# tkwa/iit

Measured on AMD Instinct MI355X. Metric: IIT (base,source) intervened pairs/sec, IOI GPT-2-small, IOI_ModelPair IIT+strict+behavior step, higher is better.
Workload: dtype bf16; 1 GPU; model=gpt2-small 12L/768d/12H (TL GPT-2 cfg, LNPre, gelu_new, V=50257), global_batch=256, seq_len=16, parallelism=dp1, engine=native, graphs=True

## Files before the change

csrc/kernels.hip:

```cpp
#include "common.h"
#include <stdlib.h>

__global__ void embed_pos_fwd_kernel(const long* __restrict__ tok, const float* __restrict__ WE,
                                     const float* __restrict__ Wpos, float* __restrict__ out, int T, int S, int d) {
  const int t = blockIdx.x;
  if (t >= T) return;
  const long v = tok[t];
  const int s = t % S;
  const float4* e = (const float4*)(WE + v * (long)d);
  const float4* p = (const float4*)(Wpos + (long)s * d);
  float4* o = (float4*)(out + (long)t * d);
  for (int i = threadIdx.x; i < d / 4; i += blockDim.x) {
    float4 a = e[i], b = p[i];
    o[i] = make_float4(a.x + b.x, a.y + b.y, a.z + b.z, a.w + b.w);
  }
}

__global__ void embed_pos_fwd_scalar_kernel(const long* __restrict__ tok, const float* __restrict__ WE,
                                            const float* __restrict__ Wpos, float* __restrict__ out, int T, int S,
                                            int d) {
  const int t = blockIdx.x;
  if (t >= T) return;
  const float* e = WE + tok[t] * (long)d;
  const float* p = Wpos + (long)(t % S) * d;
// ... 252 lines not shown
}

IIT_EXPORT int iit_attn_small_bwd(const void* qkv, const void* dz, const float* lse, void* dqkv,
                                  unsigned long long head_mask, int B, int S, int H, int dh, long ld_qkv, long ld_dz,
                                  float scale, int causal, void* stream) {
  if (S > 64 || dh > 128) return (int)hipErrorInvalidValue;
  const size_t lds = (size_t)(4 * S * (dh + 1) + 2 * S * (S + 1)) * sizeof(float);
  if (lds > kAttnSmallLdsMax) return (int)hipErrorInvalidValue;
  hipLaunchKernelGGL(attn_small_bwd_kernel, dim3(B * H), dim3(64), lds, (hipStream_t)stream, (const __bf16*)qkv,
                     (const __bf16*)dz, lse, (__bf16*)dqkv, head_mask, B, S, H, dh, ld_qkv, ld_dz, scale, causal);
  return hipGetLastError();
}

__device__ __forceinline__ void online_add(float& m, float& s, int& mi, float v, int i) {
  if (v > m) {
    s = s * __expf(m - v) + 1.f;
    m = v;
    mi = i;
  } else if (v != -INFINITY) {
    s += __expf(v - m);
  }
}

__device__ __forceinline__ void online_merge(float& m, float& s, int& mi, float om, float os, int oi) {
  if (om > m || (om == m && oi < mi)) {
    s = os + (m == -INFINITY ? 0.f : s * __expf(m - om));
    m = om;
    mi = oi;
  } else {
    s += (om == -INFINITY ? 0.f : os * __expf(om - m));
  }
}

__global__ __launch_bounds__(1024) void ce_fwd_kernel(const float* __restrict__ logits, long ld, const long* __restrict__ labels,
                                                      float* __restrict__ loss, float* __restrict__ lse_out,
                                                      long* __restrict__ amax, int V) {
  __shared__ float sm_m[16], sm_s[16];
  __shared__ int sm_i[16];
  const int row = blockIdx.x, tid = threadIdx.x, lane = tid & 63, w = tid >> 6;
  const float* x = logits + (long)row * ld;
  float m = -INFINITY, s = 0.f;
  int mi = 0x7fffffff;
  int head = 0;
  if ((((uintptr_t)x) & 15) == 0) {
    const int v4 = V / 4;
    for (int i = tid; i < v4; i += 1024) {
      const float4 q = ((const float4*)x)[i];
      online_add(m, s, mi, q.x, 4 * i);
      online_add(m, s, mi, q.y, 4 * i + 1);
      online_add(m, s, mi, q.z, 4 * i + 2);
      online_add(m, s, mi, q.w, 4 * i + 3);
    }
    head = v4 * 4;
  }
  for (int i = head + tid; i < V; i += 1024) online_add(m, s, mi, x[i], i);
#pragma unroll
  for (int o = 32; o > 0; o >>= 1) {
    const float om = __shfl_xor(m, o, 64), os = __shfl_xor(s, o, 64);
    const int oi = __shfl_xor(mi, o, 64);
    online_merge(m, s, mi, om, os, oi);
  }
  if (lane == 0) { sm_m[w] = m; sm_s[w] = s; sm_i[w] = mi; }
  __syncthreads();
  if (tid == 0) {
    for (int j = 1; j < 16; ++j) online_merge(m, s, mi, sm_m[j], sm_s[j], sm_i[j]);
    const float l = m + __logf(s);
    if (lse_out) lse_out[row] = l;
    if (loss && labels) loss[row] = l - x[labels[row]];
    if (amax) amax[row] = mi;
  }
}

IIT_EXPORT int iit_ce_fwd(const float* logits, long ld, const long* labels, float* loss, float* lse, long* amax, int R,
                          int V, void* stream) {
  hipLaunchKernelGGL(ce_fwd_kernel, dim3(R), dim3(1024), 0, (hipStream_t)stream, logits, ld, labels, loss, lse, amax, V);
  return hipGetLastError();
}

template <typename OUT>
__global__ __launch_bounds__(256) void ce_bwd_kernel(const float* __restrict__ logits, long ld, const long* __restrict__ labels,
                                                     const float* __restrict__ lse, const float* __restrict__ gscale,
                                                     float inv_rows, OUT* __restrict__ out, long ld_out, int V,
                                                     __bf16* __restrict__ out16) {
  const int row = blockIdx.y;
  const int i = blockIdx.x * 256 + threadIdx.x;
  if (i >= ld_out) return;
  float v = 0.f;
  if (i < V) {
    const float p = __expf(logits[(long)row * ld + i] - lse[row]);
    v = (p - (i == labels[row] ? 1.f : 0.f)) * gscale[0] * inv_rows;
  }
  out[(long)row * ld_out + i] = (OUT)v;
  if (out16) out16[(long)row * ld_out + i] = f2bf(v);
}

IIT_EXPORT int iit_ce_bwd(const float* logits, long ld, const long* labels, const float* lse, const float* gscale,
                          float inv_rows, void* out, long ld_out, int R, int V, int out_bf16, void* out16,
                          void* stream) {
  dim3 grid((unsigned)((ld_out + 255) / 256), R);
  if (out_bf16)
    hipLaunchKernelGGL(ce_bwd_kernel<__bf16>, grid, dim3(256), 0, (hipStream_t)stream, logits, ld, labels, lse, gscale,
                       inv_rows, (__bf16*)out, ld_out, V, (__bf16*)nullptr);
  else
    hipLaunchKernelGGL(ce_bwd_kernel<float>, grid, dim3(256), 0, (hipStream_t)stream, logits, ld, labels, lse, gscale,
                       inv_rows, (float*)out, ld_out, V, (__bf16*)out16);
  return hipGetLastError();
}

template <bool VEC>
__global__ __launch_bounds__(256) void ce_bwd16_kernel(const float* __restrict__ logits, long ld,
                                                       const long* __restrict__ labels, const float* __restrict__ lse,
                                                       const float* __restrict__ gscale, float inv_rows,
                                                       __bf16* __restrict__ out16, long ld_out, int V) {
  const int row = blockIdx.y;
  const int c0 = (blockIdx.x * 256 + threadIdx.x) * 8;
  if (c0 >= ld_out) return;
  const float* x = logits + (long)row * ld;
  const float l = lse[row], gs = gscale[0];
  const long lab = labels[row];
  float v[8];
  if (VEC && c0 + 8 <= V) {
    const float4 a = *(const float4*)(x + c0), b = *(const float4*)(x + c0 + 4);
    v[0] = a.x; v[1] = a.y; v[2] = a.z; v[3] = a.w; v[4] = b.x; v[5] = b.y; v[6] = b.z; v[7] = b.w;
  } else {
#pragma unroll
    for (int e = 0; e < 8; ++e) v[e] = c0 + e < V ? x[c0 + e] : 0.f;
  }
  bf16x8 o;
#pragma unroll
  for (int e = 0; e < 8; ++e) {
    const int i = c0 + e;
    float g = 0.f;
    if (i < V) {
      const float p = __expf(v[e] - l);
      g = (p - (i == lab ? 1.f : 0.f)) * gs * inv_rows;
    }
    o[e] = f2bf(g);
  }
  *(bf16x8*)(out16 + (long)row * ld_out + c0) = o;
}

IIT_EXPORT int iit_ce_bwd16(const float* logits, long ld, const long* labels, const float* lse, const float* gscale,
                            float inv_rows, void* out16, long ld_out, int R, int V, void* stream) {
  if (R <= 0 || V <= 0 || ld < V || ld_out < V || ld_out % 8 || ((uintptr_t)out16 & 15)) return (int)hipErrorInvalidValue;
  dim3 grid((unsigned)((ld_out / 8 + 255) / 256), R);
  const bool vec = (((uintptr_t)logits | (uintptr_t)(ld * 4)) & 15) == 0;
  if (vec)
    hipLaunchKernelGGL(ce_bwd16_kernel<true>, grid, dim3(256), 0, (hipStream_t)stream, logits, ld, labels, lse, gscale,
                       inv_rows, (__bf16*)out16, ld_out, V);
  else
    hipLaunchKernelGGL(ce_bwd16_kernel<false>, grid, dim3(256), 0, (hipStream_t)stream, logits, ld, labels, lse,
                       gscale, inv_rows, (__bf16*)out16, ld_out, V);
  return hipGetLastError();
}

struct Span {
  long start4;
  long local4;
  int len4;
  int pad;
};

__global__ __launch_bounds__(256) void sumsq_span_kernel(const float* __restrict__ g, const Span* __restrict__ spans,
                                                         int nspans, float* __restrict__ part, int do_norm,
                                                         int* __restrict__ step, float* __restrict__ gsq) {
  __shared__ float sm[4];
  if (blockIdx.x == 0 && threadIdx.x == 0 && step) step[0] += 1;
  float s = 0.f;
  if (gsq && blockIdx.x == 0 && threadIdx.x < 64) {
    s = gsq[threadIdx.x];
    gsq[threadIdx.x] = 0.f;
  }
  if (!do_norm) return;
  const float4* g4 = (const float4*)g;
  for (int e = blockIdx.x; e < nspans; e += gridDim.x) {
    const Span sp = spans[e];
    for (int i = threadIdx.x; i < sp.len4; i += 256) {
      const float4 v = g4[sp.local4 + i];
      s += (v.x * v.x + v.y * v.y) + (v.z * v.z + v.w * v.w);
    }
  }
  s = wave_sum(s);
  if ((threadIdx.x & 63) == 0) sm[threadIdx.x >> 6] = s;
  __syncthreads();
  if (threadIdx.x == 0) part[blockIdx.x] = sm[0] + sm[1] + sm[2] + sm[3];
// ... 646 lines not shown
  const int lane = threadIdx.x & 63, w = threadIdx.x >> 6;
  const float mw = wave_max(m);
  e = m == -INFINITY ? 0.f : e * __expf(m - mw);
  e = wave_sum(e);
  s = wave_sum(s);
  dba = wave_sum(dba);
  dbl = wave_sum(dbl);
  if (lane == 0) {
    red[0][w] = s; red[1][w] = mw; red[2][w] = e; red[3][w] = dba; red[4][w] = dbl;
  }
  __syncthreads();
  if (threadIdx.x == 0) {
    float M = red[1][0];
    for (int i = 1; i < 4; ++i) M = fmaxf(M, red[1][i]);
    float E = 0.f, S = 0.f, DBA = 0.f, DBL = 0.f;
    for (int i = 0; i < 4; ++i) {
      S += red[0][i];
      E += red[1][i] == -INFINITY ? 0.f : red[2][i] * __expf(red[1][i] - M);
      DBA += red[3][i];
      DBL += red[4][i];
    }
    out[4 * r + 0] = S;
    out[4 * r + 1] = M + __logf(E);
    out[4 * r + 2] = DBA;
    out[4 * r + 3] = DBL;
  }
}

IIT_EXPORT int iit_kl_rows(const float* a, long lda, const float* b, long ldb, int R, int V, float* out, void* stream) {
  if (R <= 0 || V <= 0) return 0;
  hipLaunchKernelGGL(kl_rows_kernel, dim3(R), dim3(256), 0, (hipStream_t)stream, a, lda, b, ldb, V, out);
  return hipGetLastError();
}
```

iit_amd/data/iit_dataset.py:

```python
from __future__ import annotations

from typing import Iterator, Optional, Sequence, Tuple

import numpy as np
import torch
from torch.utils.data import DataLoader, Dataset, Subset

from ..config import DEVICE


def _gather_fn(ds):
    if hasattr(ds, "gather"):
        return ds.gather
    if isinstance(ds, Subset):
        inner = _gather_fn(ds.dataset)
        if inner is None:
            return None
        table = torch.as_tensor(list(ds.indices), dtype=torch.long)
        cache = {}

        def f(idx, _inner=inner, _table=table, _cache=cache):
            dev = idx.device
            t = _cache.get(dev)
            if t is None:
                t = _cache[dev] = _table.to(dev)
            return _inner(t.index_select(0, idx))

        return f
    return None


def _dist_info() -> Tuple[int, int]:
    if torch.distributed.is_available() and torch.distributed.is_initialized():
        return torch.distributed.get_rank(), torch.distributed.get_world_size()
    return 0, 1


def loader_epoch_permutation(n: int) -> torch.Tensor:
    torch.empty((), dtype=torch.int64).random_()
    seed = int(torch.empty((), dtype=torch.int64).random_().item())
    g = torch.Generator()
    g.manual_seed(seed)
    return torch.randperm(n, generator=g)


class IITDataset(Dataset):
    def __init__(self, base_data, ablation_data, seed: int = 0, every_combination: bool = False, device=DEVICE):
        self.base_data = base_data
        self.ablation_data = ablation_data
        self.seed = seed
        self.every_combination = every_combination
        self.device = device
        self._pair_table: Optional[Tuple[np.ndarray, np.ndarray]] = None

    def pair_indices(self, index: int) -> Tuple[int, int]:
        if self.every_combination:
            n_abl = len(self.ablation_data)
            return index // n_abl, index % n_abl
        rng = np.random.default_rng(self.seed * 1000000 + index)
        base = rng.choice(len(self.base_data))
        abl = rng.choice(len(self.ablation_data))
        return int(base), int(abl)
# ... 27 lines not shown

    @staticmethod
    def collate_fn(batch, device=DEVICE):
        base, abl = zip(*batch)
        return (IITDataset.get_encoded_input_from_torch_input(base, device),
                IITDataset.get_encoded_input_from_torch_input(abl, device))

    def supports_device_loader(self) -> bool:
        return _gather_fn(self.base_data) is not None and _gather_fn(self.ablation_data) is not None

    def make_loader(self, batch_size: int, num_workers: int = 0, shuffle: bool = True, fast: Optional[bool] = None):
        if fast is None:
            fast = self.supports_device_loader()
        if fast:
            return DeviceIITLoader(self, batch_size, shuffle=shuffle)
        return DataLoader(self, batch_size=batch_size, shuffle=shuffle, num_workers=num_workers,
                          collate_fn=lambda b: self.collate_fn(b, self.device))


class DeviceIITLoader:

    def __init__(self, dataset: IITDataset, batch_size: int, shuffle: bool = True, drop_last: bool = False,
                 device=None):
        self.dataset = dataset
        self.batch_size = batch_size
        self.shuffle = shuffle
        self.drop_last = drop_last
        self.rank, self.world = _dist_info()
        self.device = torch.device(device) if device is not None else torch.device(dataset.device)
        self._base_gather = _gather_fn(dataset.base_data)
        self._abl_gather = _gather_fn(dataset.ablation_data)
        self._unique = isinstance(dataset, IITUniqueDataset)
        self._tables = None

    def _device_tables(self):
        if self._tables is None:
            if self._unique:
                self._tables = (None, None)
            else:
                b, a = self.dataset.pair_table()
                self._tables = (torch.as_tensor(b).to(self.device), torch.as_tensor(a).to(self.device))
        return self._tables

    @property
    def global_batch(self) -> int:
        return self.batch_size * self.world

    def __len__(self) -> int:
        n = len(self.dataset)
        gb = self.global_batch
        if self.drop_last or (self.world > 1 and 0 < n % gb < self.world):
            return n // gb
        return (n + gb - 1) // gb

    def __iter__(self) -> Iterator:
        n = len(self.dataset)
        perm = loader_epoch_permutation(n) if self.shuffle else torch.arange(n)
        if self.device.type == "cuda":
            perm = perm.pin_memory().to(self.device, non_blocking=True)
        else:
            perm = perm.to(self.device)
        base_t, abl_t = self._device_tables()
        gb = self.global_batch
        for start in range(0, n, gb):
            chunk = perm[start:start + gb]
            if chunk.numel() < gb and self.drop_last:
                break
            if self.world > 1:
                if chunk.numel() < self.world:
                    break
                chunk = torch.tensor_split(chunk, self.world)[self.rank]
            if self._unique:
                yield self._base_gather(chunk)
            else:
                yield (self._base_gather(base_t.index_select(0, chunk)),
                       self._abl_gather(abl_t.index_select(0, chunk)))


class IITUniqueDataset(IITDataset):

    def __getitem__(self, index):
        return self.base_data[index]

    def __len__(self) -> int:
        return len(self.base_data)

    @staticmethod
    def collate_fn(batch, device=DEVICE):
        return IITDataset.get_encoded_input_from_torch_input(batch, device)

    def supports_device_loader(self) -> bool:
        return _gather_fn(self.base_data) is not None

    def make_loader(self, batch_size: int, num_workers: int = 0, shuffle: bool = True, fast: Optional[bool] = None):
        if fast is None:
            fast = self.supports_device_loader()
        if fast:
            return DeviceIITLoader(self, batch_size, shuffle=shuffle)
        return DataLoader(self, batch_size=batch_size, shuffle=shuffle, num_workers=num_workers,
                          collate_fn=lambda b: self.collate_fn(b, self.device))


def train_test_split(dataset, test_size: float = 0.2, random_state: Optional[int] = None):
    n = len(dataset)
    split = int(n * test_size)
    if random_state is None:
# ... 4 lines not shown
```

iit_amd/model_pairs/ioi_model_pair.py:

```python
from __future__ import annotations

import numpy as np
import torch
import torch.nn.functional as F
from torch import Tensor

from ..config import DEVICE
from ..core import index as index_mod
from ..core.metric import MetricStore, MetricStoreCollection, MetricType, PerTokenMetricStore
from .base_model_pair import _ll_nodes_of
from .strict_iit_model_pair import StrictIITModelPair


def _last(t: Tensor, seq_dim_present: bool) -> Tensor:
    return t[:, -1] if seq_dim_present else t


class IOI_ModelPair(StrictIITModelPair):
    def __init__(self, hl_model, ll_model, corr, training_args=None):
        super().__init__(hl_model, ll_model, corr, training_args=training_args)
        defaults = {"next_token": False, "non_ioi_thresh": 0.65, "use_per_token_check": False}
        self.training_args = {**defaults, **self.training_args}
        self.next_token = bool(self.training_args["next_token"])

    def ll_logits_mode(self) -> str:
        return "full" if (self.next_token or not self.native()) else "last"

    def hl_run_kwargs(self):
        if self.native() and not self.next_token and getattr(self.hl_model, "supports_last_only", False):
            return {"last_only": True}
        return {}

    @property
    def loss_fn(self):
        if self._loss_fn_override is not None:
            return self._loss_fn_override
        return self.per_token_weighted_cross_entropy

    @loss_fn.setter
    def loss_fn(self, value):
        self._loss_fn_override = value

    def per_token_weighted_cross_entropy(self, output: Tensor, target: Tensor) -> Tensor:
        output = output.float()
        if output.dim() == 2:
            if target.dim() == 3 or (target.dim() == 2 and not target.dtype.is_floating_point):
                target = target[:, -1]
            if target.dtype.is_floating_point and target.dim() == 2:
                target = target.argmax(-1) if bool((target.sum(-1) == 1).all()) else target
            if not target.dtype.is_floating_point:
                from ..ops import cross_entropy
                return cross_entropy(output, target)
            return F.cross_entropy(output, target)
        if self.next_token:
            B, S, V = output.shape
            if target.dtype.is_floating_point:
                per = -(target * F.log_softmax(output, -1)).sum(-1)
            else:
                per = F.cross_entropy(output.reshape(B * S, V), target.reshape(B * S), reduction="none").view(B, S)
            w = torch.ones(S, device=output.device)
            w[-1] = 10
            return (per * w).sum() / (w.sum() * B)
        return F.cross_entropy(output[:, -1, :], target[:, -1])

    @staticmethod
    def get_label_idxs():
        return index_mod.Ix[:, -1]

    @staticmethod
    def make_test_metrics():
        return MetricStoreCollection([
            MetricStore("val/iit_loss", MetricType.LOSS),
            MetricStore("val/IIA", MetricType.ACCURACY),
            MetricStore("val/accuracy", MetricType.ACCURACY),
            PerTokenMetricStore("val/per_token_accuracy"),
        ])

    @staticmethod
    def _hl_label(hl_output: Tensor) -> Tensor:
        return torch.argmax(hl_output[:, -1] if hl_output.dim() == 3 else hl_output, dim=-1)

    def fast_hl_label(self, base_x: Tensor, ablation_x: Tensor, hl_node):
        from ..tasks.ioi.ioi_hl import IOI_HL
        hl = self.hl_model
        if not (self.native() and self.training_args.get("fast_hl", True) and type(hl) is IOI_HL
                and base_x.is_cuda and base_x.dtype == torch.long and ablation_x.dtype == torch.long):
            return None
        from ..ops import hip_kernels as K
        node = K.IOI_HL_NODES.get(hl_node.name)
        if node is None or not (hl_node.index is None or hl_node.index.is_everything()):
            return None
        if base_x.dim() != 2 or base_x.shape != ablation_x.shape or base_x.shape[1] > 64:
            return None
        if any(hp.is_live for hp in hl.hook_dict.values()):
            return None
        nm = hl.name_mover_head
# ... 65 lines not shown
```

iit_amd/model_pairs/strict_iit_model_pair.py:

```python
from __future__ import annotations

from ..core.metric import MetricStore, MetricStoreCollection, MetricType
from ..core.nodes import LLNode
from ..utils import node_picker
from .iit_behavior_model_pair import IITBehaviorModelPair


class StrictIITModelPair(IITBehaviorModelPair):
    def __init__(self, hl_model, ll_model, corr, training_args=None):
        defaults = {
            "batch_size": 256,
            "lr": 0.001,
            "num_workers": 0,
            "use_single_loss": False,
            "iit_weight": 1.0,
            "behavior_weight": 1.0,
            "strict_weight": 1.0,
            "clip_grad_norm": 1.0,
        }
        super().__init__(hl_model, ll_model, corr=corr, training_args={**defaults, **(training_args or {})})
        self.nodes_not_in_circuit = node_picker.get_nodes_not_in_circuit(self.ll_model, self.corr)

    @staticmethod
    def make_train_metrics():
        return MetricStoreCollection([
            MetricStore("train/iit_loss", MetricType.LOSS),
            MetricStore("train/behavior_loss", MetricType.LOSS),
            MetricStore("train/strict_loss", MetricType.LOSS),
        ])

    def sample_ll_node(self) -> LLNode:
        return self.rng.choice(self.nodes_not_in_circuit)

    def get_strict_loss_over_batch(self, base_input, ablation_input, ll_node: LLNode, loss_fn):
        base_x, base_y = base_input[0], base_input[1]
        out = self.ll_paired_intervention(base_x, ablation_input[0], [ll_node])
        if out is None:
            self.ll_cache = self.ll_source_cache(ablation_input[0], [ll_node])
            out = self.ll_intervened_forward(base_x, [ll_node])
        if out.dim() > 1 and out.shape[0] == 1:
            return loss_fn(out, base_y)
        return loss_fn(out.squeeze() if 1 in out.shape else out, base_y)

    def run_train_step(self, base_input, ablation_input, loss_fn, optimizer):
        args = self.training_args
        hl_node = self.sample_hl_name()

        def iit():
            return self.get_IIT_loss_over_batch(base_input, ablation_input, hl_node, loss_fn) * args["iit_weight"]

        if args["use_single_loss"]:
            ll_node = self.sample_ll_node()

            def total():
                parts = {"iit": iit(),
                         "strict": self.get_strict_loss_over_batch(base_input, ablation_input, ll_node, loss_fn)
                         * args["strict_weight"],
                         "behavior": self.get_behaviour_loss_over_batch(base_input, loss_fn) * args["behavior_weight"]}
                return parts["iit"] + parts["behavior"] + parts["strict"], parts

            _, parts = self.run_phase(("single", hl_node.name, ll_node.name, repr(ll_node.index)), total, optimizer,
                                      self.step_on_loss)
            return {"train/iit_loss": parts["iit"], "train/behavior_loss": parts["behavior"],
                    "train/strict_loss": parts["strict"]}
        iit_loss = self.run_phase(("iit", hl_node.name), iit, optimizer, self.step_on_loss)
        ll_node = self.sample_ll_node()
        strict_loss = self.run_phase(
            ("strict", ll_node.name, repr(ll_node.index)),
            lambda: self.get_strict_loss_over_batch(base_input, ablation_input, ll_node, loss_fn) * args["strict_weight"],
            optimizer, self.step_on_loss)
        behavior_loss = self.run_phase(
            ("behavior",), lambda: self.get_behaviour_loss_over_batch(base_input, loss_fn) * args["behavior_weight"],
            optimizer, self.step_on_loss)
        return {"train/iit_loss": iit_loss, "train/behavior_loss": behavior_loss, "train/strict_loss": strict_loss}
```

iit_amd/ops/__init__.py:

```python
from __future__ import annotations

from typing import Optional

import torch

from .torch_ops import TorchOps, gelu_new

_TORCH_OPS_CACHE = {}


def _torch_ops(dtype):
    ops = _TORCH_OPS_CACHE.get(dtype)
    if ops is None:
        ops = _TORCH_OPS_CACHE[dtype] = TorchOps(dtype)
    return ops


def hip_supported(cfg) -> bool:
    return (cfg.positional_embedding_type == "standard" and cfg.normalization_type in ("LN", "LNPre", None)
            and not cfg.gated_mlp and (cfg.n_key_value_heads in (None, cfg.n_heads))
            and not cfg.parallel_attn_mlp and not cfg.final_rms
            and cfg.act_fn in ("gelu_new", "gelu_fast", "gelu_pytorch_tanh", "gelu", "relu"))


def select_ops(model, backend: Optional[str] = None):
    cfg = model.cfg
    dtype = cfg.dtype
    on_gpu = next(model.parameters()).is_cuda
    if backend is None:
        from .. import config as _config
        env = _config.backend()
        backend = "hip" if (on_gpu and dtype == torch.bfloat16 and env == "hip" and hip_supported(cfg)) else "torch"
    if backend == "torch":
        return _torch_ops(dtype)
    if backend == "hip":
        if not on_gpu:
            raise RuntimeError("hip op backend requires the model on a GPU")
        from .hip_ops import get_hip_ops
        return get_hip_ops(model)
    if backend in ("hip32", "hip32x"):
        if not on_gpu:
            raise RuntimeError(f"{backend} op backend requires the model on a GPU")
        from .hip32_ops import get_hip32_ops, get_hip32x_ops
        return (get_hip32_ops if backend == "hip32" else get_hip32x_ops)(model)
    raise ValueError(f"unknown op backend {backend}")


def cross_entropy(logits: torch.Tensor, target: torch.Tensor) -> torch.Tensor:
    if logits.is_cuda and logits.dim() == 2 and not target.dtype.is_floating_point:
        from .hip_ops import cross_entropy as _hip_ce
        return _hip_ce(logits, target)
    return torch.nn.functional.cross_entropy(logits.float(), target)
```

iit_amd/ops/hip_kernels.py:

```python
from __future__ import annotations

import ctypes
import math
import os
from typing import Optional, Sequence

import numpy as np
import torch

from . import build as _build

c_void_p, c_long, c_int, c_float, c_ull = ctypes.c_void_p, ctypes.c_long, ctypes.c_int, ctypes.c_float, ctypes.c_ulonglong

EPI_BF16, EPI_BF16_BIAS3, EPI_F32_RESID, EPI_GELU, EPI_DGELU, EPI_F32_ACC, EPI_F32_ACC_QKV, EPI_F32_STORE = range(8)
EPI_GELU_ERF = 8
EPI_DGELU_ERF = 9
MODE_NN, MODE_AKM, MODE_BKM, MODE_AF32, MODE_BF32 = 0, 1, 2, 4, 8

_LIB = None
GEMM_GROUP_M = 4
GEMM_DUAL_GROUP_M = 2

_SIGS = {
    "iit_gemm": [c_void_p] * 10 + [c_long] * 5 + [c_int] * 12 + [c_void_p],
    "iit_gemm_f32": [c_void_p] * 6 + [c_long] * 4 + [c_int] * 7 + [c_void_p],
    "iit_gemm_f32_ok": [c_void_p] * 6 + [c_long] * 4 + [c_int] * 7,
    "iit_attn_f32_lds": [c_int] * 3,
    "iit_attn_f32_waves": [c_int] * 3,
    "iit_attn_f32_ok": [c_void_p] * 4 + [c_int] * 4,
    "iit_attn_f32_fwd": [c_void_p] * 6 + [c_int] * 4 + [c_float, c_int, c_void_p],
    "iit_attn_f32_bwd": [c_void_p] * 9 + [c_int] * 4 + [c_float, c_int, c_void_p],
    "iit_gemm_glds": [c_void_p] * 8 + [c_long] * 5 + [c_int] * 8 + [c_void_p] * 4,
    "iit_gemm_glds_ok": [c_void_p] * 5 + [c_long] * 5 + [c_int] * 9,
    "iit_gemm_glds_sm": [c_void_p] * 8 + [c_long] * 5 + [c_int] * 8 + [c_void_p] * 3 + [c_int] + [c_void_p] * 3,
    "iit_embed_pos_fwd": [c_void_p, c_void_p, c_void_p, c_void_p, c_int, c_int, c_int, c_void_p],
    "iit_embed_pos_bwd": [c_void_p, c_void_p, c_void_p, c_void_p, c_int, c_int, c_int, c_void_p],
    "iit_ln_fwd": [c_void_p] * 7 + [c_int, c_int, c_float, c_ull, c_int, c_int, c_void_p],
    "iit_ln_bwd": [c_void_p, c_int, c_void_p, c_int] + [c_void_p] * 10 + [c_int, c_int, c_int, c_ull, c_int, c_void_p],
    "iit_ln_bwd_part_rows": [],
    "iit_attn_small_fwd": [c_void_p] * 4 + [c_ull, c_int, c_int, c_int, c_int, c_long, c_long, c_long, c_float, c_int,
                                            c_void_p],
    "iit_attn_small_bwd": [c_void_p] * 4 + [c_ull, c_int, c_int, c_int, c_int, c_long, c_long, c_float, c_int, c_void_p],
    "iit_attn_mfma_fwd": [c_void_p] * 4 + [c_ull, c_int, c_int, c_int, c_int, c_long, c_long, c_long, c_float, c_int,
                                           c_void_p],
    "iit_attn_mfma_fwd_pair": [c_void_p] * 4 + [c_ull, c_int, c_int, c_int, c_int, c_long, c_long, c_long, c_float,
                                                c_int, c_void_p, c_int, c_ull, c_void_p],
    "iit_attn_mfma_bwd": [c_void_p] * 4 + [c_ull, c_int, c_int, c_int, c_int, c_long, c_long, c_float, c_int, c_void_p],
    "iit_attn_mfma_fwd_spec": [c_void_p] * 3 + [c_int] * 4 + [c_long, c_long, c_float, c_int, c_int, c_void_p,
                                                               c_void_p],
    "iit_attn_mfma_bwd_spec": [c_void_p] * 4 + [c_int] * 4 + [c_long, c_long, c_float, c_int, c_void_p, c_void_p],
    "iit_ce_fwd": [c_void_p, c_long, c_void_p, c_void_p, c_void_p, c_void_p, c_int, c_int, c_void_p],
    "iit_ce_bwd": [c_void_p, c_long, c_void_p, c_void_p, c_void_p, c_float, c_void_p, c_long, c_int, c_int, c_int,
                   c_void_p, c_void_p],
    "iit_gemm_glds_edge_ok": [c_void_p] * 4 + [c_long] * 3 + [c_int] * 6,
    "iit_gemm_glds_edge": [c_void_p] * 4 + [c_long] * 3 + [c_int] * 7 + [c_void_p, c_void_p, c_int, c_void_p],
    "iit_gemm_edge_plan": [c_int, c_int, c_long, c_int, c_int, c_void_p],
    "iit_ce_bwd16": [c_void_p, c_long, c_void_p, c_void_p, c_void_p, c_float, c_void_p, c_long, c_int, c_int, c_void_p],
    "iit_adam_flat": [c_void_p] * 6 + [c_int, c_void_p, c_int] + [c_float] * 6 + [c_void_p] * 3
                     + [c_void_p, c_int, c_void_p, c_void_p],
    "iit_sumsq_2d": [c_void_p, c_long, c_int, c_int, c_void_p, c_void_p],
    "iit_kl_rows": [c_void_p, c_long, c_void_p, c_long, c_int, c_int, c_void_p, c_void_p],
    "iit_adam_span_size": [],
    "iit_sumsq_spans": [c_void_p, c_void_p, c_int, c_void_p, c_int, c_int, c_void_p, c_void_p],
    "iit_adam_spans": [c_void_p] * 6 + [c_int, c_void_p] + [c_float] * 6 + [c_void_p] * 4,
    "iit_gelu_fwd": [c_void_p, c_long, c_void_p, c_long, c_int, c_int, c_int, c_void_p],
    "iit_shadow_refresh": [c_void_p, c_int, c_void_p],
    "iit_shadow_desc_size": [],
    "iit_colsum_accum": [c_void_p, c_int, c_long, c_void_p, c_int, c_int, c_void_p],
    "iit_dgelu": [c_void_p, c_void_p, c_void_p, c_long, c_int, c_void_p],
    "iit_add_bf16": [c_void_p, c_long, c_void_p, c_long, c_void_p, c_long, c_void_p, c_int, c_int, c_void_p],
    "iit_device_sync": [],
    "iit_zero_chunks": [c_void_p, c_void_p, c_int, c_void_p],
    "iit_zero_ranges": [c_void_p, c_void_p, c_void_p, c_int, c_void_p],
    "iit_colsum_multi": [c_void_p] * 6 + [c_int, c_void_p],
    "iit_rms_fwd": [c_void_p, c_int, c_void_p, c_void_p, c_void_p, c_int, c_int, c_float, c_void_p],
    "iit_rms_bwd": [c_void_p, c_void_p, c_int, c_void_p, c_void_p, c_void_p, c_void_p, c_int, c_int, c_void_p],
    "iit_rms_bwd_res": [c_void_p, c_void_p, c_int, c_void_p, c_void_p, c_void_p, c_void_p, c_void_p, c_int, c_int,
                        c_void_p],
    "iit_rotary": [c_void_p, c_long, c_long, c_long, c_void_p, c_void_p, c_void_p] + [c_int] * 8 + [c_void_p],
    "iit_swiglu_fwd": [c_void_p, c_void_p, c_void_p, c_long, c_void_p],
    "iit_swiglu_bwd": [c_void_p] * 5 + [c_long, c_void_p],
    "iit_swiglu_splice_fwd": [c_void_p] * 4 + [c_long, c_void_p, c_void_p],
    "iit_sparse_pair": [c_void_p, c_long, c_long, c_void_p, c_int, c_void_p],
    "iit_gemm_dual_set_group_m": [c_int],
    "iit_swiglu_splice_bwd": [c_void_p] * 5 + [c_long, c_void_p, c_void_p],
    "iit_embed_splice_fwd": [c_void_p, c_void_p, c_long, c_void_p, c_void_p, c_long, c_int, c_void_p, c_void_p],
    "iit_embed_splice_bwd": [c_void_p, c_void_p, c_int, c_void_p, c_long, c_long, c_int, c_void_p, c_void_p],
    "iit_flash_fwd": [c_void_p] * 3 + [c_void_p, c_void_p, c_void_p, c_void_p, c_void_p, c_void_p, c_ull] + [c_int] * 5
                     + [c_float, c_int, c_void_p, c_void_p],
    "iit_flash_bwd": [c_void_p] * 3 + [c_void_p] * 11 + [c_ull] + [c_int] * 5 + [c_float, c_int, c_void_p, c_void_p],
# ... 851 lines not shown
    _check(lib().iit_embed_splice_fwd(_p(tokens), _p(W16), W16.stride(0), _p(out), _p(src), T, d, spec_ptr,
                                      _stream()), "embed_splice_fwd")


def embed_splice_bwd(tokens, dout, grad, spec_ptr):
    T, d = tokens.numel(), dout.shape[-1]
    _check(lib().iit_embed_splice_bwd(_p(tokens), _p(dout), int(dout.dtype == torch.float32), _p(grad),
                                      grad.stride(0), T, d, spec_ptr, _stream()), "embed_splice_bwd")


def swiglu_splice_bwd(dpost, gate, up, dgate, dup, spec_ptr):
    _check(lib().iit_swiglu_splice_bwd(_p(dpost), _p(gate), _p(up), _p(dgate), _p(dup), gate.numel(), spec_ptr,
                                       _stream()), "swiglu_splice_bwd")


def swiglu_bwd(dpost, gate, up, dgate, dup):
    _check(lib().iit_swiglu_bwd(_p(dpost), _p(gate), _p(up), _p(dgate), _p(dup), gate.numel(), _stream()),
           "swiglu_bwd")


def ce_fwd(logits, ld, labels, loss, lse, amax, R, V):
    if CHECK_BOUNDS:
        _bounds("ce_fwd", ("logits", logits, R, V, ld))
    _check(lib().iit_ce_fwd(_p(logits), ld, _p(labels), _p(loss), _p(lse), _p(amax), R, V, _stream()), "ce_fwd")


def ce_bwd(logits, ld, labels, lse, gscale, inv_rows, out, ld_out, R, V, out16=None):
    if CHECK_BOUNDS:
        _bounds("ce_bwd", ("logits", logits, R, V, ld), ("out", out, R, V, ld_out))
    _check(lib().iit_ce_bwd(_p(logits), ld, _p(labels), _p(lse), _p(gscale), inv_rows, _p(out), ld_out, R, V,
                            int(out.dtype == torch.bfloat16), _p(out16), _stream()), "ce_bwd")


def ce_bwd16(logits, ld, labels, lse, gscale, inv_rows, out16, ld_out, R, V):
    assert logits.dtype == torch.float32 and out16.dtype == torch.bfloat16 and gscale.dtype == torch.float32
    if CHECK_BOUNDS:
        _bounds("ce_bwd16", ("logits", logits, R, V, ld), ("out16", out16, R, ld_out, ld_out))
    _check(lib().iit_ce_bwd16(_p(logits), ld, _p(labels), _p(lse), _p(gscale), inv_rows, _p(out16), ld_out, R, V,
                              _stream()), "ce_bwd16")


def colsum_accum(x, ld, out, T, N):
    if CHECK_BOUNDS:
        _bounds("colsum", ("x", x, T, N, ld), ("out", out, 1, N, N))
    _check(lib().iit_colsum_accum(_p(x), int(x.dtype == torch.float32), ld, _p(out), T, N, _stream()), "colsum")


def colsum_vec_ok(x, ld, out, N) -> bool:
    cpt = 4 if x.dtype == torch.float32 else 8
    return (x.dtype in (torch.float32, torch.bfloat16) and out.dtype == torch.float32 and N % cpt == 0
            and ld % cpt == 0 and x.data_ptr() % 16 == 0)


def colsum_multi(items):
    import numpy as np
    if not items:
        return
    xs = np.array([it[0].data_ptr() for it in items], dtype=np.int64)
    outs = np.array([it[2].data_ptr() for it in items], dtype=np.int64)
    lds = np.array([it[1] for it in items], dtype=np.int64)
    Ts = np.array([it[3] for it in items], dtype=np.int32)
    Ns = np.array([it[4] for it in items], dtype=np.int32)
    f32s = np.array([int(it[0].dtype == torch.float32) for it in items], dtype=np.int32)
    if CHECK_BOUNDS:
        for x, ld, out, T, N in items:
            _bounds("colsum_multi", ("x", x, T, N, ld), ("out", out, 1, N, N))
    _check(lib().iit_colsum_multi(xs.ctypes.data, outs.ctypes.data, lds.ctypes.data, Ts.ctypes.data, Ns.ctypes.data,
                                  f32s.ctypes.data, len(items), _stream()), "colsum_multi")


def colsum3_accum(x, ld, outs, T, N):
    for i, o in enumerate(outs):
# ... 70 lines not shown
```

iit_amd/ops/hip_ops.py:

```python
from __future__ import annotations

import math
import os
from typing import Optional, Sequence

import torch
from torch.autograd import Function

from ..engine import grad_hooks
from . import hip_kernels as K
from .gemm_dispatch import gemm, gemm_pair
from .torch_ops import TorchOps, act_fn

BF16 = torch.bfloat16
F32 = torch.float32


def _pad8(n: int) -> int:
    return (n + 7) // 8 * 8


def _grad_slot(p: Optional[torch.Tensor]) -> Optional[torch.Tensor]:
    if p is None or not p.requires_grad:
        return None
# ... 1036 lines not shown
        return _mlp_out_forward(ctx, pre, post, W, b, w, ldw, resid, b_in, erf)

    @staticmethod
    def backward(ctx, gy):
        if gy is None:
            return (None,) * 9
        x2, pre2 = ctx.saved_tensors
        W, b, b_in = ctx.params
        lead, Kd, N = ctx.meta
        T = x2.shape[0]
        g16 = _bf16_of(gy)
        g2 = _aligned_rows(g16, T, N)
        ldg = g2.stride(0)
        dpre = xspec = gbi = None
        if ctx.needs_input_grad[0]:
            dpre = torch.empty(T, Kd, dtype=BF16, device=g2.device)
            gbi = _grad_slot(b_in)
            xspec = dict(A=g2, B=ctx.w, C=dpre, M=T, N=Kd, K=N, lda=ldg, ldb=ctx.ldw, ldc=Kd, mode=K.MODE_NN,
                         epi=K.EPI_DGELU_ERF if ctx.erf else K.EPI_DGELU, aux=pre2, ldc2=pre2.stride(0), colsum=gbi)
        store, (gW,) = _wgrad_slots(True, W)
        gb = _grad_slot(b)
        bs = _wgrad_tail(ctx, xspec, x2, g2, ldg, (W,), *_wgrad_rows(gW, Kd, N), store, gb)
        if dpre is not None:
            dpre = dpre.view(*lead, Kd)
            if gbi is not None:
                dpre._iit_bias_sum = (dpre.data_ptr(), dpre._version, id(b_in))
        _bias_tail(bs, gb, g2, ldg, (b,), (W,))
        return dpre, None, None, None, None, None, gy, None, None


class CrossEntropyFn(Function):

    @staticmethod
    def forward(ctx, logits, labels, handle=None):
        ctx.set_materialize_grads(False)
        R, V = logits.shape
        if logits.stride(1) != 1:
            logits = logits.contiguous()
        ld = logits.stride(0)
        loss = torch.empty(R, dtype=F32, device=logits.device)
        lse = torch.empty(R, dtype=F32, device=logits.device)
        lab = labels.contiguous()
        K.ce_fwd(logits, ld, lab, loss, lse, None, R, V)
        ctx.save_for_backward(logits, lab, lse)
        ctx.only16 = handle is not None
        return loss.mean()

    @staticmethod
    def backward(ctx, g):
        if g is None:
            return None, None, None
        logits, lab, lse = ctx.saved_tensors
        R, V = logits.shape
        ld = logits.stride(0)
        ldo = _pad8(V)
        buf16 = torch.empty(R, ldo, dtype=BF16, device=logits.device)
        gs = g.reshape(1).float().contiguous()
        if ctx.only16:
            K.ce_bwd16(logits, ld, lab, lse, gs, 1.0 / R, buf16, ldo, R, V)
            return None, None, buf16[:, :V]
        buf = torch.empty(R, ldo, dtype=F32, device=logits.device)
        K.ce_bwd(logits, ld, lab, lse, gs, 1.0 / R, buf, ldo, R, V, out16=buf16)
        res = buf[:, :V]
        _set_bf16_twin(res, buf16[:, :V])
        return res, None, None


def _grad16_handle(logits: torch.Tensor) -> Optional[torch.Tensor]:
    tag = getattr(logits, "_iit_grad16", None)
    if tag is None or tag[0] != logits.data_ptr() or tag[1] != logits._version or tag[2].shape != logits.shape:
        return None
    if not (torch.is_grad_enabled() and tag[2].requires_grad) or logits._backward_hooks or logits.retains_grad:
        return None
    if os.environ.get("IIT_CE_BF16_ONLY", "1") == "0":
        return None
    return tag[2]


def cross_entropy(logits: torch.Tensor, labels: torch.Tensor) -> torch.Tensor:
    logits = logits.float()
    handle = _grad16_handle(logits) if logits.dim() == 2 else None
    if handle is not None:
        logits._iit_grad16 = None
        return CrossEntropyFn.apply(logits.detach(), labels, handle)
    return CrossEntropyFn.apply(logits, labels)




class Paired:

    __slots__ = ("base", "full", "f32")

    def __init__(self, base: torch.Tensor, full: torch.Tensor, f32=None):
        self.base, self.full, self.f32 = base, full, f32

    def resid_operands(self):
        if self.f32 is not None:
            return self.f32
        return self.base, self.full.float().contiguous()

    @property
    def nb(self) -> int:
        return self.base.shape[0]

    @property
    def src(self) -> torch.Tensor:
        return self.full[self.nb:]


class EmbedPosPairFn(EmbedPosFn):
    @staticmethod
    def forward(ctx, tokens, W_E, W_pos, tokens_full, box):
        ctx.set_materialize_grads(False)
        B2, S = tokens_full.shape
        d = W_E.shape[1]
        B = tokens.shape[0]
        out = torch.empty(B2, S, d, dtype=F32, device=tokens.device)
# ... 495 lines not shown
```

iit_amd/tasks/ioi/ioi_dataset.py:

```python
from __future__ import annotations

import random
from typing import Dict, List, Optional, Sequence

import torch
from torch.utils.data import Dataset

from ...config import DEVICE
from .ioi_config import NAMES, NOUNS, TEMPLATES, vocabulary_words
from .tokenizer import SyntheticTokenizer


def default_tokenizer() -> SyntheticTokenizer:
    return SyntheticTokenizer(vocabulary_words())


class IOIDataset(Dataset):
    def __init__(self, tokenizer=None, templates: Optional[List[str]] = None, names: Optional[List[str]] = None,
                 nouns: Optional[Dict[str, List[str]]] = None, num_samples: int = 1000, symmetric: bool = False,
                 prepend_bos: bool = True, seed: int = 42, device=None):
        self.tokenizer = tokenizer if tokenizer is not None else default_tokenizer()
        self.prepend_bos = prepend_bos
        self.templates = list(templates) if templates is not None else list(TEMPLATES)
        self.names = list(names) if names is not None else list(NAMES)
# ... 42 lines not shown
    @staticmethod
    def get_default_names():
        return list(NAMES)

    @staticmethod
    def get_default_templates():
        return list(TEMPLATES)

    @staticmethod
    def get_default_nouns():
        return {k: list(v) for k, v in NOUNS.items()}


class IOIDatasetWrapper(IOIDataset):

    def __init__(self, *args, label_format: str = "index", **kwargs):
        if label_format not in ("index", "onehot"):
            raise ValueError("label_format must be 'index' or 'onehot'")
        self.label_format = label_format
        super().__init__(*args, **kwargs)

    def _labels(self, y: torch.Tensor) -> torch.Tensor:
        if self.label_format == "onehot":
            return torch.nn.functional.one_hot(y, num_classes=self.tokenizer.vocab_size).float()
        return y

    def __getitem__(self, idx):
        p = self.prompts[idx]
        return p[:-1], self._labels(p[1:]), self.io_ids[idx:idx + 1]

    def token_ids(self) -> torch.Tensor:
        return torch.unique(self.prompts[:, :-1])

    def gather(self, idx: torch.Tensor):
        p = self.prompts.index_select(0, idx.to(self.prompts.device))
        return p[:, :-1], self._labels(p[:, 1:]), self.io_ids.index_select(0, idx.to(self.prompts.device))[:, None]
```

Measured before the change: 16990 pairs/s.

## Fuse CE mean and loss weighting into kernels; fuse pair batch gather

The cross-entropy forward gains a mean variant. The last block to finish, found through an atomic ticket, reduces the per-row losses and applies the loss weight, which replaces a separate mean launch and weight multiply. The backward folds the weight into the bf16 gradient kernel. A new kernel gathers base and source prompts, labels and IO ids for a batch in one launch, replacing several index_select and slicing ops per batch. The ticket-based last-block reduction adds cross-block atomic ordering to get right and a shared per-device ticket buffer.

```diff
diff --git a/csrc/kernels.hip b/csrc/kernels.hip
--- a/csrc/kernels.hip
+++ b/csrc/kernels.hip
@@ -308,9 +308,11 @@
   }
 }
 
+template <bool MEAN>
 __global__ __launch_bounds__(1024) void ce_fwd_kernel(const float* __restrict__ logits, long ld, const long* __restrict__ labels,
                                                       float* __restrict__ loss, float* __restrict__ lse_out,
-                                                      long* __restrict__ amax, int V) {
+                                                      long* __restrict__ amax, int V, float weight,
+                                                      float* __restrict__ mean_out, int* __restrict__ ticket) {
   __shared__ float sm_m[16], sm_s[16];
   __shared__ int sm_i[16];
   const int row = blockIdx.x, tid = threadIdx.x, lane = tid & 63, w = tid >> 6;
@@ -342,14 +344,59 @@
     for (int j = 1; j < 16; ++j) online_merge(m, s, mi, sm_m[j], sm_s[j], sm_i[j]);
     const float l = m + __logf(s);
     if (lse_out) lse_out[row] = l;
-    if (loss && labels) loss[row] = l - x[labels[row]];
+    if constexpr (MEAN) {
+      __hip_atomic_store(loss + row, l - x[labels[row]], __ATOMIC_RELAXED, __HIP_MEMORY_SCOPE_AGENT);
+    } else {
+      if (loss && labels) loss[row] = l - x[labels[row]];
+    }
     if (amax) amax[row] = mi;
+  }
+  if constexpr (MEAN) {
+    __shared__ int is_last;
+    const int R = gridDim.x;
+    if (tid == 0) {
+      asm volatile("s_waitcnt vmcnt(0)" ::: "memory");
+      const int last = __hip_atomic_fetch_add(ticket, 1, __ATOMIC_RELAXED, __HIP_MEMORY_SCOPE_AGENT) == R - 1;
+      if (last) __hip_atomic_store(ticket, 0, __ATOMIC_RELAXED, __HIP_MEMORY_SCOPE_AGENT);
+      is_last = last;
+    }
+    __syncthreads();
+    if (!is_last) return;
+    float acc = 0.f;
+    for (int base = 0; base < R; base += 4096) {
+      float v[4];
+#pragma unroll
+      for (int e = 0; e < 4; ++e) {
+        const int i = base + e * 1024 + tid;
+        v[e] = i < R ? __hip_atomic_load(loss + i, __ATOMIC_RELAXED, __HIP_MEMORY_SCOPE_AGENT) : 0.f;
+      }
+      acc += (v[0] + v[1]) + (v[2] + v[3]);
+    }
+#pragma unroll
+    for (int o = 32; o > 0; o >>= 1) acc += __shfl_xor(acc, o, 64);
+    if (lane == 0) sm_s[w] = acc;
+    __syncthreads();
+    if (w == 0) {
+      float t = lane < 16 ? sm_s[lane] : 0.f;
+#pragma unroll
+      for (int o = 8; o > 0; o >>= 1) t += __shfl_xor(t, o, 64);
+      if (lane == 0) mean_out[0] = t / (float)R * weight;
+    }
   }
 }
 
 IIT_EXPORT int iit_ce_fwd(const float* logits, long ld, const long* labels, float* loss, float* lse, long* amax, int R,
                           int V, void* stream) {
-  hipLaunchKernelGGL(ce_fwd_kernel, dim3(R), dim3(1024), 0, (hipStream_t)stream, logits, ld, labels, loss, lse, amax, V);
+  hipLaunchKernelGGL(ce_fwd_kernel<false>, dim3(R), dim3(1024), 0, (hipStream_t)stream, logits, ld, labels, loss, lse,
+                     amax, V, 1.f, (float*)nullptr, (int*)nullptr);
+  return hipGetLastError();
+}
+
+IIT_EXPORT int iit_ce_fwd_mean(const float* logits, long ld, const long* labels, float* loss, float* lse, int R, int V,
+                               float weight, float* mean_out, int* ticket, void* stream) {
+  if (R <= 0 || V <= 0 || ld < V || !labels || !loss || !mean_out || !ticket) return (int)hipErrorInvalidValue;
+  hipLaunchKernelGGL(ce_fwd_kernel<true>, dim3(R), dim3(1024), 0, (hipStream_t)stream, logits, ld, labels, loss, lse,
+                     (long*)nullptr, V, weight, mean_out, ticket);
   return hipGetLastError();
 }
 
@@ -386,13 +433,14 @@
 template <bool VEC>
 __global__ __launch_bounds__(256) void ce_bwd16_kernel(const float* __restrict__ logits, long ld,
                                                        const long* __restrict__ labels, const float* __restrict__ lse,
-                                                       const float* __restrict__ gscale, float inv_rows,
-                                                       __bf16* __restrict__ out16, long ld_out, int V) {
+                                                       const float* __restrict__ gscale, float weight,
+                                                       float inv_rows, __bf16* __restrict__ out16, long ld_out,
+                                                       int V) {
   const int row = blockIdx.y;
   const int c0 = (blockIdx.x * 256 + threadIdx.x) * 8;
   if (c0 >= ld_out) return;
   const float* x = logits + (long)row * ld;
-  const float l = lse[row], gs = gscale[0];
+  const float l = lse[row], gs = gscale[0] * weight;
   const long lab = labels[row];
   float v[8];
   if (VEC && c0 + 8 <= V) {
@@ -417,16 +465,16 @@
 }
 
 IIT_EXPORT int iit_ce_bwd16(const float* logits, long ld, const long* labels, const float* lse, const float* gscale,
-                            float inv_rows, void* out16, long ld_out, int R, int V, void* stream) {
+                            float inv_rows, void* out16, long ld_out, int R, int V, float weight, void* stream) {
   if (R <= 0 || V <= 0 || ld < V || ld_out < V || ld_out % 8 || ((uintptr_t)out16 & 15)) return (int)hipErrorInvalidValue;
   dim3 grid((unsigned)((ld_out / 8 + 255) / 256), R);
   const bool vec = (((uintptr_t)logits | (uintptr_t)(ld * 4)) & 15) == 0;
   if (vec)
     hipLaunchKernelGGL(ce_bwd16_kernel<true>, grid, dim3(256), 0, (hipStream_t)stream, logits, ld, labels, lse, gscale,
-                       inv_rows, (__bf16*)out16, ld_out, V);
+                       weight, inv_rows, (__bf16*)out16, ld_out, V);
   else
     hipLaunchKernelGGL(ce_bwd16_kernel<false>, grid, dim3(256), 0, (hipStream_t)stream, logits, ld, labels, lse,
-                       gscale, inv_rows, (__bf16*)out16, ld_out, V);
+                       gscale, weight, inv_rows, (__bf16*)out16, ld_out, V);
   return hipGetLastError();
 }
 
@@ -1139,3 +1187,41 @@
   hipLaunchKernelGGL(kl_rows_kernel, dim3(R), dim3(256), 0, (hipStream_t)stream, a, lda, b, ldb, V, out);
   return hipGetLastError();
 }
+
+struct PairGatherSide {
+  const long* tab;
+  const long* prompts;
+  const long* io;
+  long* x;
+  long* y;
+  long* iv;
+  long N;
+};
+
+__global__ __launch_bounds__(256) void pair_batch_gather_kernel(const long* __restrict__ perm, int n, long ntab, int S1,
+                                                                const PairGatherSide a, const PairGatherSide b) {
+  const PairGatherSide& sd = blockIdx.y == 0 ? a : b;
+  const int e = blockIdx.x * 256 + threadIdx.x;
+  if (e >= n * S1) return;
+  const int r = e / S1, c = e - r * S1, S = S1 - 1;
+  const long p = perm[r];
+  if ((unsigned long)p >= (unsigned long)ntab) return;
+  const long i = sd.tab[p];
+  if ((unsigned long)i >= (unsigned long)sd.N) return;
+  const long v = sd.prompts[i * S1 + c];
+  if (c < S) sd.x[(long)r * S + c] = v;
+  if (c > 0) sd.y[(long)r * S + c - 1] = v;
+  if (c == 0) sd.iv[r] = sd.io[i];
+}
+
+IIT_EXPORT int iit_pair_batch_gather(const long* perm, int n, long ntab, int S1, const long* tab_b, const long* prompts_b,
+                                     const long* io_b, long Nb, const long* tab_a, const long* prompts_a,
+                                     const long* io_a, long Na, long* xb, long* yb, long* ivb, long* xa, long* ya,
+                                     long* iva, void* stream) {
+  if (n <= 0) return 0;
+  if (S1 < 2 || (long)n * S1 > 0x7fffffffL) return (int)hipErrorInvalidValue;
+  const PairGatherSide a{tab_b, prompts_b, io_b, xb, yb, ivb, Nb}, b{tab_a, prompts_a, io_a, xa, ya, iva, Na};
+  hipLaunchKernelGGL(pair_batch_gather_kernel, dim3((unsigned)(((long)n * S1 + 255) / 256), 2), dim3(256), 0,
+                     (hipStream_t)stream, perm, n, ntab, S1, a, b);
+  return hipGetLastError();
+}
diff --git a/iit_amd/data/iit_dataset.py b/iit_amd/data/iit_dataset.py
--- a/iit_amd/data/iit_dataset.py
+++ b/iit_amd/data/iit_dataset.py
@@ -28,6 +28,21 @@
 
         return f
     return None
+
+
+def _pair_gather_side(ds, table: torch.Tensor):
+    while isinstance(ds, Subset):
+        table = torch.as_tensor(list(ds.indices), dtype=torch.long).to(table.device).index_select(0, table)
+        ds = ds.dataset
+    ops = ds.pair_gather_operands() if hasattr(ds, "pair_gather_operands") else None
+    if ops is None:
+        return None
+    prompts, io_ids = ops
+    if prompts.device != table.device or prompts.dtype != torch.long or io_ids.dtype != torch.long:
+        return None
+    if table.numel() and not (0 <= int(table.min()) and int(table.max()) < prompts.shape[0]):
+        raise IndexError("pair table points outside the dataset")
+    return table.contiguous(), prompts.contiguous(), io_ids.contiguous()
 
 
 def _dist_info() -> Tuple[int, int]:
@@ -121,6 +136,7 @@
         self._abl_gather = _gather_fn(dataset.ablation_data)
         self._unique = isinstance(dataset, IITUniqueDataset)
         self._tables = None
+        self._sides = None
 
     def _device_tables(self):
         if self._tables is None:
@@ -131,6 +147,18 @@
                 self._tables = (torch.as_tensor(b).to(self.device), torch.as_tensor(a).to(self.device))
         return self._tables
 
+    def _pair_sides(self):
+        if self._sides is None:
+            sides = None
+            if self.device.type == "cuda" and not self._unique:
+                ds = self.dataset
+                sides = tuple(_pair_gather_side(d, t) for d, t in zip((ds.base_data, ds.ablation_data),
+                                                                      self._device_tables()))
+                if None in sides or sides[0][1].shape[1] != sides[1][1].shape[1]:
+                    sides = None
+            self._sides = (sides,)
+        return self._sides[0]
+
     @property
     def global_batch(self) -> int:
         return self.batch_size * self.world
@@ -150,6 +178,7 @@
         else:
             perm = perm.to(self.device)
         base_t, abl_t = self._device_tables()
+        sides = self._pair_sides()
         gb = self.global_batch
         for start in range(0, n, gb):
             chunk = perm[start:start + gb]
@@ -161,6 +190,9 @@
                 chunk = torch.tensor_split(chunk, self.world)[self.rank]
             if self._unique:
                 yield self._base_gather(chunk)
+            elif sides is not None:
+                from ..ops import hip_kernels
+                yield hip_kernels.pair_batch_gather(chunk, sides[0], sides[1], sides[0][1].shape[1])
             else:
                 yield (self._base_gather(base_t.index_select(0, chunk)),
                        self._abl_gather(abl_t.index_select(0, chunk)))
diff --git a/iit_amd/model_pairs/ioi_model_pair.py b/iit_amd/model_pairs/ioi_model_pair.py
--- a/iit_amd/model_pairs/ioi_model_pair.py
+++ b/iit_amd/model_pairs/ioi_model_pair.py
@@ -41,7 +41,13 @@
     def loss_fn(self, value):
         self._loss_fn_override = value
 
-    def per_token_weighted_cross_entropy(self, output: Tensor, target: Tensor) -> Tensor:
+    def per_token_weighted_cross_entropy(self, output: Tensor, target: Tensor, weight=None) -> Tensor:
+        if weight is not None:
+            if output.dim() == 2 and output.is_cuda and (
+                    not target.dtype.is_floating_point and target.dim() in (1, 2)):
+                from ..ops import cross_entropy
+                return cross_entropy(output.float(), target[:, -1] if target.dim() == 2 else target, weight=weight)
+            return self.per_token_weighted_cross_entropy(output, target) * weight
         output = output.float()
         if output.dim() == 2:
             if target.dim() == 3 or (target.dim() == 2 and not target.dtype.is_floating_point):
@@ -62,6 +68,8 @@
             w[-1] = 10
             return (per * w).sum() / (w.sum() * B)
         return F.cross_entropy(output[:, -1, :], target[:, -1])
+
+    per_token_weighted_cross_entropy.takes_weight = True
 
     @staticmethod
     def get_label_idxs():
diff --git a/iit_amd/model_pairs/strict_iit_model_pair.py b/iit_amd/model_pairs/strict_iit_model_pair.py
--- a/iit_amd/model_pairs/strict_iit_model_pair.py
+++ b/iit_amd/model_pairs/strict_iit_model_pair.py
@@ -42,21 +42,29 @@
             return loss_fn(out, base_y)
         return loss_fn(out.squeeze() if 1 in out.shape else out, base_y)
 
+    @staticmethod
+    def _weighted(loss_fn, weight):
+        if getattr(loss_fn, "takes_weight", False) and isinstance(weight, (int, float)):
+            return lambda out, y: loss_fn(out, y, weight=float(weight))
+        return lambda out, y: loss_fn(out, y) * weight
+
     def run_train_step(self, base_input, ablation_input, loss_fn, optimizer):
         args = self.training_args
         hl_node = self.sample_hl_name()
+        iit_fn = self._weighted(loss_fn, args["iit_weight"])
+        strict_fn = self._weighted(loss_fn, args["strict_weight"])
+        behavior_fn = self._weighted(loss_fn, args["behavior_weight"])
 
         def iit():
-            return self.get_IIT_loss_over_batch(base_input, ablation_input, hl_node, loss_fn) * args["iit_weight"]
+            return self.get_IIT_loss_over_batch(base_input, ablation_input, hl_node, iit_fn)
 
         if args["use_single_loss"]:
             ll_node = self.sample_ll_node()
 
             def total():
                 parts = {"iit": iit(),
-                         "strict": self.get_strict_loss_over_batch(base_input, ablation_input, ll_node, loss_fn)
-                         * args["strict_weight"],
-                         "behavior": self.get_behaviour_loss_over_batch(base_input, loss_fn) * args["behavior_weight"]}
+                         "strict": self.get_strict_loss_over_batch(base_input, ablation_input, ll_node, strict_fn),
+                         "behavior": self.get_behaviour_loss_over_batch(base_input, behavior_fn)}
                 return parts["iit"] + parts["behavior"] + parts["strict"], parts
 
             _, parts = self.run_phase(("single", hl_node.name, ll_node.name, repr(ll_node.index)), total, optimizer,
@@ -67,9 +75,9 @@
         ll_node = self.sample_ll_node()
         strict_loss = self.run_phase(
             ("strict", ll_node.name, repr(ll_node.index)),
-            lambda: self.get_strict_loss_over_batch(base_input, ablation_input, ll_node, loss_fn) * args["strict_weight"],
+            lambda: self.get_strict_loss_over_batch(base_input, ablation_input, ll_node, strict_fn),
             optimizer, self.step_on_loss)
         behavior_loss = self.run_phase(
-            ("behavior",), lambda: self.get_behaviour_loss_over_batch(base_input, loss_fn) * args["behavior_weight"],
+            ("behavior",), lambda: self.get_behaviour_loss_over_batch(base_input, behavior_fn),
             optimizer, self.step_on_loss)
         return {"train/iit_loss": iit_loss, "train/behavior_loss": behavior_loss, "train/strict_loss": strict_loss}
diff --git a/iit_amd/ops/__init__.py b/iit_amd/ops/__init__.py
--- a/iit_amd/ops/__init__.py
+++ b/iit_amd/ops/__init__.py
@@ -46,8 +46,9 @@
     raise ValueError(f"unknown op backend {backend}")
 
 
-def cross_entropy(logits: torch.Tensor, target: torch.Tensor) -> torch.Tensor:
+def cross_entropy(logits: torch.Tensor, target: torch.Tensor, weight: Optional[float] = None) -> torch.Tensor:
     if logits.is_cuda and logits.dim() == 2 and not target.dtype.is_floating_point:
         from .hip_ops import cross_entropy as _hip_ce
-        return _hip_ce(logits, target)
-    return torch.nn.functional.cross_entropy(logits.float(), target)
+        return _hip_ce(logits, target, weight)
+    loss = torch.nn.functional.cross_entropy(logits.float(), target)
+    return loss if weight is None else loss * weight
diff --git a/iit_amd/ops/hip_kernels.py b/iit_amd/ops/hip_kernels.py
--- a/iit_amd/ops/hip_kernels.py
+++ b/iit_amd/ops/hip_kernels.py
@@ -55,7 +55,12 @@
     "iit_gemm_glds_edge_ok": [c_void_p] * 4 + [c_long] * 3 + [c_int] * 6,
     "iit_gemm_glds_edge": [c_void_p] * 4 + [c_long] * 3 + [c_int] * 7 + [c_void_p, c_void_p, c_int, c_void_p],
     "iit_gemm_edge_plan": [c_int, c_int, c_long, c_int, c_int, c_void_p],
-    "iit_ce_bwd16": [c_void_p, c_long, c_void_p, c_void_p, c_void_p, c_float, c_void_p, c_long, c_int, c_int, c_void_p],
+    "iit_ce_bwd16": [c_void_p, c_long, c_void_p, c_void_p, c_void_p, c_float, c_void_p, c_long, c_int, c_int, c_float,
+                     c_void_p],
+    "iit_ce_fwd_mean": [c_void_p, c_long, c_void_p, c_void_p, c_void_p, c_int, c_int, c_float, c_void_p, c_void_p,
+                        c_void_p],
+    "iit_pair_batch_gather": [c_void_p, c_int, c_long, c_int, c_void_p, c_void_p, c_void_p, c_long, c_void_p, c_void_p,
+                              c_void_p, c_long] + [c_void_p] * 7,
     "iit_adam_flat": [c_void_p] * 6 + [c_int, c_void_p, c_int] + [c_float] * 6 + [c_void_p] * 3
                      + [c_void_p, c_int, c_void_p, c_void_p],
     "iit_sumsq_2d": [c_void_p, c_long, c_int, c_int, c_void_p, c_void_p],
@@ -973,12 +978,50 @@
                             int(out.dtype == torch.bfloat16), _p(out16), _stream()), "ce_bwd")
 
 
-def ce_bwd16(logits, ld, labels, lse, gscale, inv_rows, out16, ld_out, R, V):
+def ce_bwd16(logits, ld, labels, lse, gscale, inv_rows, out16, ld_out, R, V, weight: float = 1.0):
     assert logits.dtype == torch.float32 and out16.dtype == torch.bfloat16 and gscale.dtype == torch.float32
     if CHECK_BOUNDS:
         _bounds("ce_bwd16", ("logits", logits, R, V, ld), ("out16", out16, R, ld_out, ld_out))
     _check(lib().iit_ce_bwd16(_p(logits), ld, _p(labels), _p(lse), _p(gscale), inv_rows, _p(out16), ld_out, R, V,
-                              _stream()), "ce_bwd16")
+                              float(weight), _stream()), "ce_bwd16")
+
+
+_CE_TICKETS = {}
+
+
+def ce_ticket(device) -> torch.Tensor:
+    t = _CE_TICKETS.get(device)
+    if t is None:
+        t = _CE_TICKETS[device] = torch.zeros(1, dtype=torch.int32, device=device)
+    return t
+
+
+def ce_fwd_mean(logits, ld, labels, loss, lse, R, V, weight: float, mean_out, ticket=None):
+    assert logits.dtype == torch.float32 and labels.dtype == torch.long and labels.is_contiguous()
+    assert loss.dtype == torch.float32 and loss.numel() >= R and mean_out.dtype == torch.float32
+    if ticket is None:
+        ticket = ce_ticket(logits.device)
+    assert ticket.dtype == torch.int32
+    if CHECK_BOUNDS:
+        _bounds("ce_fwd_mean", ("logits", logits, R, V, ld))
+    _check(lib().iit_ce_fwd_mean(_p(logits), ld, _p(labels), _p(loss), _p(lse), R, V, float(weight), _p(mean_out),
+                                 _p(ticket), _stream()), "ce_fwd_mean")
+
+
+def pair_batch_gather(perm, base, source, S1: int):
+    n, dev = perm.numel(), perm.device
+    ntab = base[0].numel()
+    for tab, prompts, io in (base, source):
+        for t in (perm, tab, prompts, io):
+            if t.dtype != torch.long or not t.is_contiguous() or t.device != dev:
+                raise ValueError("pair_batch_gather: operands must be contiguous int64 tensors on one device")
+        if tab.numel() != ntab or prompts.dim() != 2 or prompts.shape[1] != S1 or io.numel() != prompts.shape[0]:
+            raise ValueError("pair_batch_gather: table / prompt / io shapes do not match")
+    out = [torch.empty(n, w, dtype=torch.long, device=dev) for w in (S1 - 1, S1 - 1, 1) * 2]
+    _check(lib().iit_pair_batch_gather(_p(perm), n, ntab, S1, _p(base[0]), _p(base[1]), _p(base[2]), base[1].shape[0],
+                                       _p(source[0]), _p(source[1]), _p(source[2]), source[1].shape[0],
+                                       *[_p(t) for t in out], _stream()), "pair_batch_gather")
+    return tuple(out[:3]), tuple(out[3:])
 
 
 def colsum_accum(x, ld, out, T, N):
diff --git a/iit_amd/ops/hip_ops.py b/iit_amd/ops/hip_ops.py
--- a/iit_amd/ops/hip_ops.py
+++ b/iit_amd/ops/hip_ops.py
@@ -1092,7 +1092,7 @@
 class CrossEntropyFn(Function):
 
     @staticmethod
-    def forward(ctx, logits, labels, handle=None):
+    def forward(ctx, logits, labels, handle=None, weight=None):
         ctx.set_materialize_grads(False)
         R, V = logits.shape
         if logits.stride(1) != 1:
@@ -1101,15 +1101,22 @@
         loss = torch.empty(R, dtype=F32, device=logits.device)
         lse = torch.empty(R, dtype=F32, device=logits.device)
         lab = labels.contiguous()
+        ctx.only16 = handle is not None
+        ctx.weight = 1.0 if weight is None else float(weight)
+        if weight is not None:
+            assert handle is not None
+            out = torch.empty((), dtype=F32, device=logits.device)
+            K.ce_fwd_mean(logits, ld, lab, loss, lse, R, V, ctx.weight, out)
+            ctx.save_for_backward(logits, lab, lse)
+            return out
         K.ce_fwd(logits, ld, lab, loss, lse, None, R, V)
         ctx.save_for_backward(logits, lab, lse)
-        ctx.only16 = handle is not None
         return loss.mean()
 
     @staticmethod
     def backward(ctx, g):
         if g is None:
-            return None, None, None
+            return None, None, None, None
         logits, lab, lse = ctx.saved_tensors
         R, V = logits.shape
         ld = logits.stride(0)
@@ -1117,13 +1124,13 @@
         buf16 = torch.empty(R, ldo, dtype=BF16, device=logits.device)
         gs = g.reshape(1).float().contiguous()
         if ctx.only16:
-            K.ce_bwd16(logits, ld, lab, lse, gs, 1.0 / R, buf16, ldo, R, V)
-            return None, None, buf16[:, :V]
+            K.ce_bwd16(logits, ld, lab, lse, gs, 1.0 / R, buf16, ldo, R, V, weight=ctx.weight)
+            return None, None, buf16[:, :V], None
         buf = torch.empty(R, ldo, dtype=F32, device=logits.device)
         K.ce_bwd(logits, ld, lab, lse, gs, 1.0 / R, buf, ldo, R, V, out16=buf16)
         res = buf[:, :V]
         _set_bf16_twin(res, buf16[:, :V])
-        return res, None, None
+        return res, None, None, None
 
 
 def _grad16_handle(logits: torch.Tensor) -> Optional[torch.Tensor]:
@@ -1137,13 +1144,17 @@
     return tag[2]
 
 
-def cross_entropy(logits: torch.Tensor, labels: torch.Tensor) -> torch.Tensor:
+def cross_entropy(logits: torch.Tensor, labels: torch.Tensor, weight: Optional[float] = None) -> torch.Tensor:
     logits = logits.float()
     handle = _grad16_handle(logits) if logits.dim() == 2 else None
     if handle is not None:
         logits._iit_grad16 = None
-        return CrossEntropyFn.apply(logits.detach(), labels, handle)
-    return CrossEntropyFn.apply(logits, labels)
+        if weight is not None and labels.dtype == torch.long:
+            return CrossEntropyFn.apply(logits.detach(), labels, handle, float(weight))
+        loss = CrossEntropyFn.apply(logits.detach(), labels, handle)
+    else:
+        loss = CrossEntropyFn.apply(logits, labels)
+    return loss if weight is None else loss * weight
 
 
 
diff --git a/iit_amd/tasks/ioi/ioi_dataset.py b/iit_amd/tasks/ioi/ioi_dataset.py
--- a/iit_amd/tasks/ioi/ioi_dataset.py
+++ b/iit_amd/tasks/ioi/ioi_dataset.py
@@ -98,6 +98,11 @@
     def token_ids(self) -> torch.Tensor:
         return torch.unique(self.prompts[:, :-1])
 
+    def pair_gather_operands(self):
+        if self.label_format != "index" or not self.prompts.is_cuda or self.prompts.shape[1] < 2:
+            return None
+        return self.prompts, self.io_ids
+
     def gather(self, idx: torch.Tensor):
         p = self.prompts.index_select(0, idx.to(self.prompts.device))
         return p[:, :-1], self._labels(p[:, 1:]), self.io_ids.index_select(0, idx.to(self.prompts.device))[:, None]
```

Measured after the change: 17010 pairs/s (median of 5 runs). No clear change (+0.2%).
